# NVIDIA-Merlin/distributed-embeddings

Measured on NVIDIA H100. Metric: DLRM global samples/sec (device-timed, max over ranks), higher is better.
Workload: dtype bf16

## Files before the change

distributed_embeddings_b200/models/dlrm_fast.py:

```python
from __future__ import annotations

import os
from typing import Optional

import torch
from torch import nn

from ..ops import _native
from ..parallel.comm import CommContext
from ..parallel.fused import FusedEngine
from ..utils import nvtx
from ..utils.lr_schedule import LearningRateScheduler
from ..utils.metrics import BinnedAUC, auc_from_histogram
from .dense_optimizer import FlatDenseOptimizer, dense_optimizer_config
from .dlrm import DLRM


def _pad8(n: int) -> int:
  return (n + 7) // 8 * 8


class _Layer:

  def __init__(self, lin: nn.Linear, relu: bool):
    self.lin = lin
    self.relu = relu
    self.out_f, self.in_f = lin.weight.shape
    self.in_pad = _pad8(self.in_f)
    self.w_off = self.b_off = 0
    self.w_numel = self.out_f * self.in_pad
    self.b_numel = _pad8(self.out_f)


class DLRMTrainStep:

  def __init__(self, model: DLRM, lr: float = 24.0, embedding_optimizer: str = "sgd",
               scheduler: Optional[LearningRateScheduler] = None, use_cuda_graph: bool = True,
               embedding_optimizer_kwargs: Optional[dict] = None, overlap: bool = True,
               gemm: str = "cublas", eval_thresholds: int = 8000, dense_optimizer: str = "sgd",
               dense_optimizer_kwargs: Optional[dict] = None):
    if gemm not in ("cublas", "fused_dgrad", "tcgen05", "tcgen05_pair"):
      raise ValueError("gemm must be cublas | fused_dgrad | tcgen05 | tcgen05_pair")
    self.gemm = gemm
    self.dense_cfg = dense_optimizer_config(dense_optimizer, dense_optimizer_kwargs)
    self.model = model
    self.emb = model.embedding
    if self.emb.backend != "fused":
      raise ValueError("DLRMTrainStep needs the fused embedding back end")
    self.dev = self.emb.device
    self.ops = _native.require()
    self.world = self.emb.world_size
    self.ctx = CommContext.for_group(self.emb.group, self.dev)
    self.scheduler = scheduler
    self.use_cuda_graph = use_cuda_graph
    self.overlap = overlap
    self.emb.set_optimizer(embedding_optimizer, lr=lr, **(embedding_optimizer_kwargs or {}))
    if self.emb._engine is None:
      self.emb._engine = FusedEngine(self.emb)
    self.engine: FusedEngine = self.emb._engine
    self.n_emb = len(model.table_sizes)
    self.dim = model.embedding_dim
    sp_env = os.environ.get("DE_B200_STREAM_PUSH", "auto")
    self._stream_push = self.world > 1 and (sp_env == "1" or (sp_env == "auto" and self.world >= 4))
    self._push_stream = torch.cuda.Stream(device=self.dev) if self._stream_push else None
    self._push_ready = torch.cuda.Event() if self._stream_push else None

# ... 178 lines not shown
    H = self.head
    ops.head_loss(last.y, H.w16.view(-1), H.b16, self.lab_in, 1.0 / b, last.dy,
                  H.gw.view(-1), H.gb, last.gb, self.loss, None)
    for i in range(len(self.top) - 1, -1, -1):
      L = self.top[i]
      x = self.top[i - 1].y if i > 0 else self.z
      dx = self.top[i - 1].dy if i > 0 else self.dz
      self._wgrad(L, x)
      if i > 0:
        self._dgrad_relu(L, x, dx, self.top[i - 1].gb)
      else:
        torch.mm(L.dy, L.w16, out=dx)
    if self._ar_stream is not None:
      ar = self._ar_stream
      ar.wait_stream(torch.cuda.current_stream())
      if getattr(self, "_w_used", False):
        ar.wait_stream(self._wstream)
      off = self.top[0].w_off
      with torch.cuda.stream(ar):
        self.ctx.allreduce_(self.gsym, self.n_flat - off, torch.float32, scale=1.0 / self.world,
                            byte_offset=off * 4, max_blocks=32)
    hb = self.bottom[-1]
    pushed = eng.streamed_push
    if pushed:
      eng.push_counters.zero_()
      self._push_ready.record(torch.cuda.current_stream())
      ops.interact_bwd(hb.y, eng.out, self.n_emb, self.dz, hb.dy, 0, 0, 1.0, eng.routes_stage,
                       len(eng.routes_stage_np), [], eng.push_counters, eng.push_chunk_rows)
      self._push_stream.wait_event(self._push_ready)
      with torch.cuda.stream(self._push_stream):
        eng.launch_streamed_push()
    else:
      ops.interact_bwd(hb.y, eng.out, self.n_emb, self.dz, hb.dy, 0, 0, 1.0, eng.routes_all,
                       len(eng.routes_all_np), eng.sync_grad_signal(), None, 0)
    if self._side is not None:
      self._side.wait_stream(torch.cuda.current_stream())
      if pushed:
        self._side.wait_stream(self._push_stream)
      with torch.cuda.stream(self._side):
        eng.backward_inplace()
    else:
      if pushed:
        torch.cuda.current_stream().wait_stream(self._push_stream)
      eng.backward_inplace()
    ops.relu_bwd_bias(hb.dy, hb.y, hb.gb)
    for i in range(len(self.bottom) - 1, -1, -1):
      L = self.bottom[i]
      x = self.bottom[i - 1].y if i > 0 else self.x0
      self._wgrad(L, x)
      if i > 0:
        self._dgrad_relu(L, x, self.bottom[i - 1].dy, self.bottom[i - 1].gb)
    if self._dp_slots and self._side is not None:
      torch.cuda.current_stream().wait_stream(self._side)
    if getattr(self, "_w_used", False):
      torch.cuda.current_stream().wait_stream(self._wstream)
      self._w_used = False
    if self.world > 1:
      if self._ar_stream is not None:
        ar = self._ar_stream
        ar.wait_stream(torch.cuda.current_stream())
        with torch.cuda.stream(ar):
          self.ctx.allreduce_(self.gsym, self.top[0].w_off, torch.float32, scale=1.0 / self.world)
        torch.cuda.current_stream().wait_stream(ar)
      else:
        self.ctx.allreduce_(self.gsym, self.n_flat, torch.float32, scale=1.0 / self.world)
    self.dense_opt.apply(ops, self.p16, self.g32, self.lr_t)
    self._refresh_transposes()
# ... 181 lines not shown
```

distributed_embeddings_b200/ops/csrc/bindings.cpp:

```cpp
#include <ATen/cuda/CUDAContext.h>
#include <c10/cuda/CUDAGuard.h>
#include <c10/cuda/CUDAStream.h>
#include <cuda_runtime.h>
#include <torch/library.h>
#include <torch/torch.h>

#include <cstdlib>
#include <cstring>
#include <mutex>
#include <string>
#include <unordered_map>
#include <vector>

#include "de_b200.h"

namespace {

using at::Tensor;

#define DE_CUDA_CHECK(expr)                                                              \
  do {                                                                                   \
    cudaError_t _e = (expr);                                                             \
    TORCH_CHECK(_e == cudaSuccess, "CUDA error in " #expr ": ", cudaGetErrorString(_e)); \
  } while (0)
// ... 714 lines not shown
  check_bf16_2d(bottom, "bottom");
  check_bf16_2d(emb, "emb");
  check_bf16_2d(z, "z");
  c10::cuda::CUDAGuard guard(bottom.device());
  const int64_t dim = bottom.size(1);
  TORCH_CHECK(emb.size(1) == n_emb * dim, "emb must be [batch, n_emb * dim]");
  TORCH_CHECK(emb.size(0) >= bottom.size(0) && z.size(0) >= bottom.size(0),
              "emb and z need a row per row of bottom");
  check_row_alignment(bottom, 16, "bottom");
  check_row_alignment(emb, 16, "emb");
  const int64_t need = (n_emb + 1) * n_emb / 2 + dim;
  TORCH_CHECK(z.size(1) >= need, "z is too narrow");
  bool ok = de::launch_interact_fwd(bottom.data_ptr(), bottom.stride(0), emb.data_ptr(),
                                    emb.stride(0), static_cast<int>(n_emb), static_cast<int>(dim),
                                    z.data_ptr(), z.stride(0), static_cast<int>(z.size(1)),
                                    bottom.size(0), sm_count(), cur_stream(), to_sync(sync));
  TORCH_CHECK(ok, "unsupported interaction shape (n_emb <= 31, dim in {16,32,64,128})");
  check_launch();
}

void interact_bwd(const Tensor& bottom, const Tensor& emb, int64_t n_emb, const Tensor& dz,
                  Tensor dbottom, int64_t demb_ptr, int64_t demb_stride, double emb_grad_scale,
                  const c10::optional<Tensor>& routes, int64_t n_routes, at::IntArrayRef sync,
                  const c10::optional<Tensor>& done_counters, int64_t chunk_rows) {
  check_bf16_2d(bottom, "bottom");
  check_bf16_2d(emb, "emb");
  check_bf16_2d(dz, "dz");
  check_bf16_2d(dbottom, "dbottom");
  if (routes.has_value()) {
    TORCH_CHECK(routes->is_cuda() && routes->scalar_type() == at::kByte &&
                routes->numel() >= n_routes * static_cast<int64_t>(sizeof(de::GradRoute)));
  } else {
    TORCH_CHECK(demb_ptr != 0, "interact_bwd needs an embedding-gradient buffer or routes");
  }
  const int64_t dim = bottom.size(1);
  const int64_t batch = bottom.size(0);
  TORCH_CHECK(emb.size(1) == n_emb * dim, "emb must be [batch, n_emb * dim]");
  TORCH_CHECK((n_emb + 1) * n_emb / 2 + dim <= dz.size(1), "dz is too narrow");
  TORCH_CHECK(dbottom.size(1) == dim, "dbottom must be [batch, dim]");
  TORCH_CHECK(emb.size(0) >= batch && dz.size(0) >= batch && dbottom.size(0) >= batch,
              "emb, dz and dbottom need a row per row of bottom");
  check_row_alignment(bottom, 16, "bottom");
  check_row_alignment(emb, 16, "emb");
  check_row_alignment(dbottom, 4, "dbottom");
  if (!routes.has_value())
    TORCH_CHECK(demb_stride % 2 == 0 && demb_ptr % 4 == 0,
                "embedding-gradient rows must start on 4-byte boundaries");
  if (done_counters.has_value()) {
    TORCH_CHECK(done_counters->is_cuda() && done_counters->scalar_type() == at::kInt &&
                    done_counters->is_contiguous(),
                "done_counters must be a contiguous int32 CUDA tensor");
    TORCH_CHECK(chunk_rows > 0, "chunk_rows must be positive with done_counters");
    TORCH_CHECK(done_counters->numel() >= (batch + chunk_rows - 1) / chunk_rows,
                "done_counters needs one counter per chunk of chunk_rows samples");
  }
  c10::cuda::CUDAGuard guard(bottom.device());
  bool ok = de::launch_interact_bwd(bottom.data_ptr(), bottom.stride(0), emb.data_ptr(),
                                    emb.stride(0), static_cast<int>(n_emb), static_cast<int>(dim),
                                    dz.data_ptr(), dz.stride(0), dbottom.data_ptr(),
                                    dbottom.stride(0), reinterpret_cast<void*>(demb_ptr),
                                    demb_stride, static_cast<float>(emb_grad_scale),
                                    bottom.size(0), sm_count(), cur_stream(),
                                    routes.has_value()
                                        ? reinterpret_cast<const de::GradRoute*>(routes->data_ptr())
                                        : nullptr,
                                    static_cast<int>(n_routes), to_sync(sync),
                                    done_counters.has_value()
                                        ? reinterpret_cast<uint32_t*>(done_counters->data_ptr<int>())
                                        : nullptr,
                                    static_cast<int>(chunk_rows));
  TORCH_CHECK(ok, "unsupported interaction shape (n_emb <= 31, dim in {32,64,128}; routed / "
                  "signalling launches need dim in {64,128} and 16-byte aligned rows)");
  check_launch();
}

void avgpool_fwd(const Tensor& x, int64_t n, Tensor out, int64_t stride) {
  check_bf16_2d(x, "x");
  check_bf16_2d(out, "out");
  const int64_t out_len = (n + stride - 1) / stride;
  TORCH_CHECK(x.size(1) >= n && out.size(1) >= out_len && out.size(0) == x.size(0));
  const int64_t pad = std::max<int64_t>(0, (out_len - 1) * stride + stride - n);
  c10::cuda::CUDAGuard guard(x.device());
  de::launch_avgpool_fwd(x.data_ptr(), x.stride(0), static_cast<int>(n), out.data_ptr(),
                         out.stride(0), static_cast<int>(out_len), static_cast<int>(stride),
                         static_cast<int>(pad / 2), x.size(0), cur_stream());
  check_launch();
}

void avgpool_bwd(const Tensor& dout, Tensor dx, int64_t n, int64_t stride) {
  check_bf16_2d(dout, "dout");
  check_bf16_2d(dx, "dx");
  const int64_t out_len = (n + stride - 1) / stride;
  TORCH_CHECK(dx.size(1) >= n && dout.size(1) >= out_len && dout.size(0) == dx.size(0));
// ... 327 lines not shown
      "-> ()",
      &push_grad);
  m.def(
      "stream_push(int[] src_ptrs, int[] dst_ptrs, int[] row_bytes, Tensor counters, "
      "int chunk_rows, int rows, int blocks, int[] sync) -> ()",
      &stream_push);
  m.def(
      "rowslice_reduce(Tensor partial, int out_ptr, int out_stride, int out_dtype, Tensor cols) "
      "-> ()",
      &rowslice_reduce);
  m.def(
      "gather_ragged(Tensor segs, int[] val_ptrs, int[] split_ptrs, Tensor(a!) dst_vals, "
      "Tensor(b!) goff, int b, int max_cap) -> ()",
      &gather_ragged);
  m.def("select_copy(Tensor[] src0, Tensor[] src1, Tensor(a!)[] dst, Tensor slot_flag) -> ()",
        &select_copy);
  m.def("copy_cast_2d(Tensor src, int dst_ptr, int dst_stride, int dst_dtype, float scale) -> ()",
        &copy_cast_2d);
  m.def("interact_fwd(Tensor bottom, Tensor emb, int n_emb, Tensor(a!) z, int[] sync) -> ()",
        &interact_fwd);
  m.def(
      "interact_bwd(Tensor bottom, Tensor emb, int n_emb, Tensor dz, Tensor(a!) dbottom, "
      "int demb_ptr, int demb_stride, float emb_grad_scale, Tensor? routes, int n_routes, "
      "int[] sync, Tensor? done_counters, int chunk_rows) -> ()",
      &interact_bwd);
  m.def("avgpool_fwd(Tensor x, int n, Tensor(a!) out, int stride) -> ()", &avgpool_fwd);
  m.def("avgpool_bwd(Tensor dout, Tensor(a!) dx, int n, int stride) -> ()", &avgpool_bwd);
  m.def("relu_bwd_bias(Tensor(a!) dy, Tensor y, Tensor(b!) db) -> ()", &relu_bwd_bias);
  m.def(
      "head_loss(Tensor x, Tensor w, Tensor bias, Tensor labels, float inv_batch, Tensor(a!) dx, "
      "Tensor(b!) dw, Tensor(c!) db, Tensor(d!) dbias_prev, Tensor(e!) loss_sum, Tensor? logits) "
      "-> ()",
      &head_loss);
  m.def(
      "head_eval(Tensor x, Tensor w, Tensor bias, Tensor labels, Tensor n_valid, Tensor(a!) probs, "
      "Tensor(b!) hist, Tensor(c!) loss_sum, Tensor(d!) count) -> ()",
      &head_eval);
  m.def(
      "dense_sgd(Tensor(a!) p32, Tensor(b!) p16, Tensor(c!) g32, Tensor lr, float grad_scale) "
      "-> ()",
      &dense_sgd);
  m.def(
      "dense_adagrad(Tensor(a!) p32, Tensor(b!) p16, Tensor(c!) g32, Tensor(d!) acc, Tensor lr, "
      "float eps) -> ()",
      &dense_adagrad);
  m.def(
      "dense_adam(Tensor(a!) p32, Tensor(b!) p16, Tensor(c!) g32, Tensor(d!) m, Tensor(e!) v, "
// ... 18 lines not shown
```

distributed_embeddings_b200/ops/csrc/de_b200.h:

```cpp
#pragma once
#include <cuda_runtime.h>
#include <stdint.h>

namespace de {

constexpr int kMaxPeers = 16;
constexpr int kGridCapSms = 132;

struct alignas(16) InputDesc {
  const void* table;
  const void* ids;
  const int64_t* offsets;
  int64_t ids_off;
  int64_t id_shift;
  int64_t sub_rows;
  int64_t row_base;
  int32_t width;
  int32_t hotness;
  int32_t dst_col;
  int32_t combiner;
  int32_t local_table;
  int32_t flags;
  int64_t item_off;
};
// ... 139 lines not shown
};
void launch_stream_push(const PushPlan& plan, const uint32_t* counters, int chunk_rows,
                        int64_t rows, unsigned long long timeout, int* error_flag, int blocks,
                        cudaStream_t stream, const SyncArgs& sync);
void launch_rowslice_reduce(const float* partial, int world, int64_t rows, int64_t part_stride,
                            void* out, int64_t out_stride, int out_dtype, const int32_t* cols,
                            int n_cols, cudaStream_t stream);
void launch_gather_segments(const int64_t* segs, int n_seg, const PeerPtrs& src, void* dst,
                            int elem_bytes, int64_t max_seg_elems, cudaStream_t stream);
void launch_gather_ragged(const int64_t* segs, int n_seg, const PeerPtrs& src_vals,
                          const PeerPtrs& src_splits, void* dst_vals, int64_t* goff, int64_t b,
                          int world, int elem_bytes, int64_t max_cap, cudaStream_t stream);
void launch_select_copy(const void* const* src0, const void* const* src1, void* const* dst,
                        const int64_t* nbytes, int count, const int* slot_flag, int sm_count,
                        cudaStream_t stream);
void launch_copy_cast_2d(const void* src, int64_t src_stride, void* dst, int64_t dst_stride,
                         int64_t rows, int64_t cols, int src_dtype, int dst_dtype, float scale,
                         cudaStream_t stream);

bool launch_interact_fwd(const void* bottom, int64_t bottom_stride, const void* emb,
                         int64_t emb_stride, int n_emb, int dim, void* z, int64_t z_stride,
                         int z_width, int64_t batch, int sm_count, cudaStream_t stream,
                         const SyncArgs& sync);
bool launch_interact_bwd(const void* bottom, int64_t bottom_stride, const void* emb,
                         int64_t emb_stride, int n_emb, int dim, const void* dz,
                         int64_t dz_stride, void* dbottom, int64_t dbottom_stride, void* demb,
                         int64_t demb_stride, float emb_grad_scale, int64_t batch, int sm_count,
                         cudaStream_t stream, const GradRoute* routes, int n_routes,
                         const SyncArgs& sync, uint32_t* done_counters = nullptr,
                         int chunk_rows = 0);
void launch_avgpool_fwd(const void* x, int64_t x_stride, int n, void* out, int64_t out_stride,
                        int out_len, int stride, int left, int64_t rows, cudaStream_t stream);
void launch_avgpool_bwd(const void* dout, int64_t dout_stride, int out_len, void* dx,
                        int64_t dx_stride, int n, int stride, int left, int64_t rows,
                        cudaStream_t stream);
void launch_relu_bwd_bias(void* dy, const void* y, float* db, int64_t rows, int cols,
                          cudaStream_t stream);
bool launch_head_loss(const void* x, int K, const void* w, const void* bias, const float* labels,
                      int64_t batch, float inv_batch, void* dx, float* dw, float* db,
                      float* dbias_prev, float* loss_sum, float* logits_out, int sm_count,
                      cudaStream_t stream);
bool launch_head_eval(const void* x, int K, const void* w, const void* bias, const float* labels,
                      int64_t batch, const int64_t* n_valid, float* probs, int64_t* hist, int nb,
                      double* loss_sum, int64_t* count, int sm_count, cudaStream_t stream);
void launch_sgd_update(float* p32, void* p16, float* g32, const float* lr_ptr, float grad_scale,
                       int64_t n, int sm_count, cudaStream_t stream);
bool launch_dense_opt(int kind, float* p32, void* p16, float* g32, float* s0, float* s1,
                      const float* lr_ptr, const float* step_ptr, float beta1, float beta2,
                      float eps, int64_t n, int sm_count, cudaStream_t stream);
void launch_cast_pad(const float* src, int src_cols, void* dst, int dst_cols, int64_t rows,
                     cudaStream_t stream);

bool launch_gemm_tn_fused(const void* A, int64_t lda, const void* B, int64_t ldb, const void* bias,
// ... 9 lines not shown
```

distributed_embeddings_b200/ops/csrc/dense_kernels.cu:

```cuda
#include <cuda_bf16.h>
#include <cuda_runtime.h>
#include <stdint.h>

#include <cstdlib>

#include "common.cuh"
#include "de_b200.h"

namespace de {

namespace {

using bf16 = __nv_bfloat16;

__device__ __forceinline__ uint32_t smem_u32(const void* p) {
  return static_cast<uint32_t>(__cvta_generic_to_shared(p));
}

__device__ __forceinline__ void ldmatrix_x4(uint32_t (&r)[4], uint32_t addr) {
  asm volatile("ldmatrix.sync.aligned.m8n8.x4.shared.b16 {%0,%1,%2,%3}, [%4];"
               : "=r"(r[0]), "=r"(r[1]), "=r"(r[2]), "=r"(r[3])
               : "r"(addr));
}
__device__ __forceinline__ void ldmatrix_x4_trans(uint32_t (&r)[4], uint32_t addr) {
// ... 217 lines not shown

constexpr int kDzMax = 512;

template <int D>
__device__ __forceinline__ void issue_sample(bf16* sF, int LD, bf16* sDz, const bf16* bottom,
                                             const bf16* emb, const bf16* dz, int n_emb,
                                             int dz_chunks, int lane) {
  constexpr int kChunks = D / 8;
  const int total = (n_emb + 1) * kChunks;
#pragma unroll 4
  for (int c = lane; c < total; c += 32) {
    const int row = c / kChunks, ch = c - row * kChunks;
    const bf16* src = row == 0 ? bottom + ch * 8 : emb + (row - 1) * D + ch * 8;
    cp_async16(sF + row * LD + ch * 8, src);
  }
  for (int c = lane; c < dz_chunks; c += 32) cp_async16(sDz + c * 8, dz + c * 8);
}

struct ChunkDst {
  unsigned long long base;
  long long stride;
};

template <int D>
__global__ void __launch_bounds__(kWarps * 32)
interact_bwd_v2_kernel(const bf16* __restrict__ bottom, int64_t bottom_stride,
                       const bf16* __restrict__ emb, int64_t emb_stride, int n_emb,
                       const bf16* __restrict__ dz, int64_t dz_stride, bf16* __restrict__ dbottom,
                       int64_t dbottom_stride, bf16* __restrict__ demb, int64_t demb_stride,
                       float emb_grad_scale, int64_t batch,
                       const GradRoute* __restrict__ routes, int n_routes,
                       const __grid_constant__ SyncArgs sync, uint32_t* __restrict__ done_counters,
                       int chunk_rows) {
  constexpr int LD = D + 8;
  constexpr int LDG = 40;
  constexpr int kWarpElems = 2 * kMaxFeat * LD + 2 * kDzMax + kMaxFeat * LDG;
  constexpr int kRowChunks = D / 8;
  extern __shared__ __align__(16) unsigned char smem_raw[];
  const int warp = threadIdx.x >> 5, lane = threadIdx.x & 31;
  bf16* base = reinterpret_cast<bf16*>(smem_raw) + warp * kWarpElems;
  bf16* sDz0 = base + 2 * kMaxFeat * LD;
  bf16* sG = sDz0 + 2 * kDzMax;
  ChunkDst* sDst = reinterpret_cast<ChunkDst*>(reinterpret_cast<bf16*>(smem_raw) +
                                               kWarps * kWarpElems);
  const int nf = n_emb + 1;
  const int n_inter = nf * (nf - 1) / 2;
  const int dz_chunks = (n_inter + D + 7) >> 3;
  const int n_chunks = n_emb * kRowChunks;
  if (routes == nullptr) {
    for (int c = threadIdx.x; c < n_chunks; c += blockDim.x) {
      sDst[c].base = reinterpret_cast<unsigned long long>(demb + c * 8);
      sDst[c].stride = demb_stride * 2;
    }
  } else {
    for (int r = 0; r < n_routes; ++r) {
      const GradRoute R = routes[r];
      const int c0 = R.src_col >> 3, nc = R.width >> 3;
      for (int c = threadIdx.x; c < nc; c += blockDim.x) {
        sDst[c0 + c].base =
            reinterpret_cast<unsigned long long>(reinterpret_cast<bf16*>(R.dst) + R.dst_col + c * 8);
        sDst[c0 + c].stride = R.dst_stride * 2;
      }
    }
  }
  zero_pad_rows<D>(base, LD, n_emb, lane);
  zero_pad_rows<D>(base + kMaxFeat * LD, LD, n_emb, lane);
  __syncthreads();

  const int64_t stride = static_cast<int64_t>(gridDim.x) * kWarps;
  int64_t s = static_cast<int64_t>(blockIdx.x) * kWarps + warp;
  int cur = 0;
  if (s < batch)
    issue_sample<D>(base, LD, sDz0, bottom + s * bottom_stride, emb + s * emb_stride,
                    dz + s * dz_stride, n_emb, dz_chunks, lane);
  cp_async_commit();
  for (; s < batch; s += stride, cur ^= 1) {
    const int64_t nxt = s + stride;
    if (nxt < batch)
      issue_sample<D>(base + (cur ^ 1) * (kMaxFeat * LD), LD, sDz0 + (cur ^ 1) * kDzMax,
                      bottom + nxt * bottom_stride, emb + nxt * emb_stride, dz + nxt * dz_stride,
                      n_emb, dz_chunks, lane);
    cp_async_commit();
    cp_async_wait_group<1>();
    __syncwarp();
    bf16* sF = base + cur * (kMaxFeat * LD);
    const bf16* sDz = sDz0 + cur * kDzMax;
    for (int c = lane; c < kMaxFeat * LDG / 8; c += 32)
      reinterpret_cast<uint4*>(sG)[c] = make_uint4(0, 0, 0, 0);
    __syncwarp();
    for (int idx = lane; idx < n_inter; idx += 32) {
      int i = static_cast<int>((1.0f + sqrtf(1.0f + 8.0f * idx)) * 0.5f);
      while (i * (i - 1) / 2 > idx) --i;
      while ((i + 1) * i / 2 <= idx) ++i;
      const int j = idx - i * (i - 1) / 2;
      const bf16 v = sDz[idx];
      sG[i * LDG + j] = v;
      sG[j * LDG + i] = v;
    }
    __syncwarp();
    uint32_t ga[2][2][4];
#pragma unroll
    for (int mt = 0; mt < 2; ++mt)
#pragma unroll
      for (int ks = 0; ks < 2; ++ks)
// ... 22 lines not shown
      for (int mt = 0; mt < 2; ++mt) {
#pragma unroll
        for (int nt = 0; nt < 4; ++nt) {
#pragma unroll
          for (int half = 0; half < 2; ++half) {
            const int row = mt * 16 + cr + half * 8;
            const int col = n0 + nt * 8 + cc;
            float v0 = acc[mt][nt][half * 2], v1 = acc[mt][nt][half * 2 + 1];
            if (row == 0) {
              v0 += __bfloat162float(sDz[n_inter + col]);
              v1 += __bfloat162float(sDz[n_inter + col + 1]);
            } else {
              v0 *= emb_grad_scale;
              v1 *= emb_grad_scale;
            }
            if (row <= n_emb)
              *reinterpret_cast<__nv_bfloat162*>(sF + row * LD + col) =
                  __floats2bfloat162_rn(v0, v1);
          }
        }
      }
    }
    __syncwarp();
    if (lane < kRowChunks)
      *reinterpret_cast<uint4*>(dbottom + s * dbottom_stride + lane * 8) =
          *reinterpret_cast<const uint4*>(sF + lane * 8);
    for (int c = lane; c < n_chunks; c += 32) {
      const int row = 1 + c / kRowChunks, ch = c - (row - 1) * kRowChunks;
      const ChunkDst d = sDst[c];
      *reinterpret_cast<uint4*>(d.base + static_cast<unsigned long long>(s * d.stride)) =
          *reinterpret_cast<const uint4*>(sF + row * LD + ch * 8);
    }
    __syncwarp();
    if (done_counters != nullptr && lane == 0) {
      __threadfence();
      atomicAdd(done_counters + s / chunk_rows, 1u);
    }
  }
  cp_async_wait_group<0>();
  sync_tail(sync);
}

constexpr int kRbUnroll = 4;
__global__ void __launch_bounds__(256)
relu_bwd_bias_kernel(bf16* __restrict__ dy, const bf16* __restrict__ y, float* __restrict__ db,
                     int64_t rows, int cols, int rows_per_block) {
  extern __shared__ float s_part[];
  const int tpr = cols >> 3;
  const int rows_par = blockDim.x / tpr;
  const int tr = threadIdx.x / tpr, tc = threadIdx.x - tr * tpr;
  const int64_t r0 = static_cast<int64_t>(blockIdx.x) * rows_per_block;
  const int64_t r1 = min(rows, r0 + rows_per_block);
  float acc[8] = {0, 0, 0, 0, 0, 0, 0, 0};
  if (tr < rows_par) {
    for (int64_t r = r0 + tr; r < r1; r += static_cast<int64_t>(rows_par) * kRbUnroll) {
      uint4 g[kRbUnroll], a[kRbUnroll];
#pragma unroll
      for (int u = 0; u < kRbUnroll; ++u) {
        const int64_t rr = r + static_cast<int64_t>(u) * rows_par;
        if (rr < r1) {
          g[u] = *reinterpret_cast<const uint4*>(dy + rr * cols + tc * 8);
          a[u] = *reinterpret_cast<const uint4*>(y + rr * cols + tc * 8);
        }
// ... 328 lines not shown
#define DE_IFWD(DD)                                                                              \
  {                                                                                              \
    const size_t smem = kWarps * fwd_warp_bytes(DD);                                             \
    cudaFuncSetAttribute(interact_fwd_kernel<DD>, cudaFuncAttributeMaxDynamicSharedMemorySize,   \
                         static_cast<int>(smem));                                                \
    interact_fwd_kernel<DD><<<static_cast<unsigned>(blocks), kWarps * 32, smem, stream>>>(       \
        reinterpret_cast<const bf16*>(bottom), bottom_stride, reinterpret_cast<const bf16*>(emb), \
        emb_stride, n_emb, reinterpret_cast<bf16*>(z), z_stride, z_width, batch, sync);          \
    return true;                                                                                 \
  }
  if (dim == 128) DE_IFWD(128)
  if (dim == 64) DE_IFWD(64)
  if (dim == 32) DE_IFWD(32)
  if (dim == 16) DE_IFWD(16)
#undef DE_IFWD
  return false;
}

bool launch_interact_bwd(const void* bottom, int64_t bottom_stride, const void* emb,
                         int64_t emb_stride, int n_emb, int dim, const void* dz,
                         int64_t dz_stride, void* dbottom, int64_t dbottom_stride, void* demb,
                         int64_t demb_stride, float emb_grad_scale, int64_t batch, int sm_count,
                         cudaStream_t stream, const GradRoute* routes, int n_routes,
                         const SyncArgs& sync, uint32_t* done_counters, int chunk_rows) {
  if (n_emb + 1 > kMaxFeat || batch <= 0 || dim % 32 != 0) return false;
  int64_t blocks = (batch + kWarps - 1) / kWarps;
  const int64_t cap = static_cast<int64_t>(sm_count) * 8;
  if (blocks > cap) blocks = cap;
  static const bool force_v1 = [] {
    const char* v = std::getenv("DE_B200_INTERACT_V1");
    return v != nullptr && v[0] == '1';
  }();
  const int nf = n_emb + 1;
  const int dz_elems = (nf * (nf - 1) / 2 + dim + 7) / 8 * 8;
  const bool v2_ok =
      dz_elems <= kDzMax && dz_elems <= dz_stride && dz_stride % 8 == 0 &&
      bottom_stride % 8 == 0 && emb_stride % 8 == 0 && dbottom_stride % 8 == 0 &&
      ((reinterpret_cast<uintptr_t>(dz) | reinterpret_cast<uintptr_t>(bottom) |
        reinterpret_cast<uintptr_t>(emb) | reinterpret_cast<uintptr_t>(dbottom)) & 15) == 0 &&
      (dim == 128 || dim == 64) &&
      (routes != nullptr || (demb_stride % 8 == 0 && (reinterpret_cast<uintptr_t>(demb) & 15) == 0));
  if ((routes != nullptr || done_counters != nullptr) && !v2_ok) return false;
  const bool has_sync = sync.state != nullptr && (sync.wait_ch >= 0 || sync.signal_ch >= 0);
  if (v2_ok && (!force_v1 || routes != nullptr || has_sync || done_counters != nullptr)) {
    int64_t blocks2 = (batch + kWarps - 1) / kWarps;
    if (blocks2 > static_cast<int64_t>(sm_count) * 2) blocks2 = static_cast<int64_t>(sm_count) * 2;
#define DE_IBWD2(DD)                                                                             \
  {                                                                                              \
    const size_t smem =                                                                          \
        kWarps * (2 * kMaxFeat * (DD + 8) + 2 * kDzMax + kMaxFeat * 40) * sizeof(bf16) +         \
        static_cast<size_t>(n_emb) * (DD / 8) * sizeof(ChunkDst);                                \
    cudaFuncSetAttribute(interact_bwd_v2_kernel<DD>,                                             \
                         cudaFuncAttributeMaxDynamicSharedMemorySize, static_cast<int>(smem));   \
    interact_bwd_v2_kernel<DD><<<static_cast<unsigned>(blocks2), kWarps * 32, smem, stream>>>(   \
        reinterpret_cast<const bf16*>(bottom), bottom_stride, reinterpret_cast<const bf16*>(emb), \
        emb_stride, n_emb, reinterpret_cast<const bf16*>(dz), dz_stride,                         \
        reinterpret_cast<bf16*>(dbottom), dbottom_stride, reinterpret_cast<bf16*>(demb),         \
        demb_stride, emb_grad_scale, batch, routes, n_routes, sync, done_counters, chunk_rows);  \
    return true;                                                                                 \
  }
    if (dim == 128) DE_IBWD2(128)
    if (dim == 64) DE_IBWD2(64)
#undef DE_IBWD2
  }
  if (has_sync) return false;
#define DE_IBWD(DD)                                                                              \
  {                                                                                              \
    const size_t smem = kWarps * (kMaxFeat * (DD + 8) + kMaxFeat * 40) * sizeof(bf16);           \
    cudaFuncSetAttribute(interact_bwd_kernel<DD>, cudaFuncAttributeMaxDynamicSharedMemorySize,   \
                         static_cast<int>(smem));                                                \
    interact_bwd_kernel<DD><<<static_cast<unsigned>(blocks), kWarps * 32, smem, stream>>>(       \
        reinterpret_cast<const bf16*>(bottom), bottom_stride, reinterpret_cast<const bf16*>(emb), \
        emb_stride, n_emb, reinterpret_cast<const bf16*>(dz), dz_stride,                         \
        reinterpret_cast<bf16*>(dbottom), dbottom_stride, reinterpret_cast<bf16*>(demb),         \
        demb_stride, emb_grad_scale, batch);                                                     \
    return true;                                                                                 \
  }
  if (dim == 128) DE_IBWD(128)
  if (dim == 64) DE_IBWD(64)
  if (dim == 32) DE_IBWD(32)
#undef DE_IBWD
  return false;
}

void launch_relu_bwd_bias(void* dy, const void* y, float* db, int64_t rows, int cols,
// ... 104 lines not shown
```

distributed_embeddings_b200/parallel/dry_run.py:

```python
from __future__ import annotations

import bisect
import ctypes
import threading
from typing import Dict, List, Optional, Sequence, Tuple

import numpy as np
import torch

from ..ops._native import GRAD_ROUTE, INPUT_DESC, MAX_PEERS, TABLE_DESC
from ..ops.stochastic_rounding import stochastic_round
from . import fused as _fused


class DryWorld:

  def __init__(self, world_size: int):
    self.world_size = int(world_size)
    self.lock = threading.Lock()
    self._barrier = threading.Barrier(self.world_size)
    self._bufs: Dict[Tuple[int, int], torch.Tensor] = {}
    self._ranges: Dict[int, int] = {}
    self._starts: List[int] = []
    self._keep: List[torch.Tensor] = []
# ... 336 lines not shown
    self._count("scatter_add_bwd")
    self._wait(sync)
    if staged:
      esz = 4 if int(act_dtype) == 0 else 2
      assert (grad_stride * esz) % 16 == 0 and all(int(p) % 16 == 0 for p in grad_ptrs)
      for d in self._descs(descs, n_inputs):
        rb = int(d["width"]) * esz
        assert rb % 16 == 0 and rb <= 256 and (int(d["dst_col"]) * esz) % 16 == 0
    if scale_ptr:
      scale = scale * float(self.world.tensor(int(scale_ptr), torch.float32, 1, "lr")[0])
    for d in self._descs(descs, n_inputs):
      table = self._table(d)
      for dd in range(-(-batch // grad_batch)):
        g0, g1 = dd * grad_batch, min(batch, (dd + 1) * grad_batch)
        vals, lens = self._ids_of(d, g0, g1, ids64, src_ptrs, src_batch)
        ids = vals + int(d["id_shift"])
        ok = (ids >= 0) & (ids < int(d["sub_rows"]))
        g = self._grad_rows(d, dd, g1 - g0, grad_ptrs, grad_stride, act_dtype)
        w = torch.full((g1 - g0,), float(scale))
        if int(d["combiner"]) == 1:
          w = w / lens.clamp(min=1).to(w.dtype)
        per_id = (g * w.unsqueeze(1))[self._pool_index(lens)]
        table.index_add_(0, int(d["row_base"]) + ids[ok], per_id[ok])

  def sort_items(self, descs, tables, n_tables, n_inputs, batch, src_batch, src_ptrs, ids64,
                 n_items, total_rows, prefill_sentinel):
    self._count("sort_items")
    D = self._descs(descs, n_inputs)
    T = self._descs(tables, n_tables, TABLE_DESC)
    keys = torch.full((n_items,), int(total_rows), dtype=torch.int64)
    items = torch.zeros(n_items, dtype=torch.int64)
    covered = torch.zeros(n_items, dtype=torch.bool)
    for f, d in enumerate(D):
      vals, lens = self._ids_of(d, 0, batch, ids64, src_ptrs, src_batch)
      ids = vals + int(d["id_shift"])
      ok = (ids >= 0) & (ids < int(d["sub_rows"]))
      key = int(T[int(d["local_table"])]["key_base"]) + int(d["row_base"]) + ids
      key = torch.where(ok, key, torch.full_like(key, int(total_rows)))
      first = int(d["item_off"])
      if int(d["offsets"]):
        offs = self.world.tensor(int(d["offsets"]), torch.int64, batch + 1, "csr offsets")
        first += int(offs[0])
      n = key.numel()
      assert first + n <= n_items, "item range outside the sort buffers"
      assert not bool(covered[first:first + n].any()), "item ranges of two inputs overlap"
      covered[first:first + n] = True
# ... 152 lines not shown
```

distributed_embeddings_b200/parallel/fused.py:

```python
from __future__ import annotations

import os
import weakref
from typing import Any, Dict, List, Optional, Sequence, Tuple

import numpy as np
import torch

from ..ops import _native
from ..ops._native import DTYPE_CODE, GRAD_ROUTE, INPUT_DESC, TABLE_DESC
from ..ops.ragged import RaggedIds
from ..utils import nvtx
from .comm import CH_BARRIER0, CH_CONSUMED, CH_GRAD, CH_IDS, CH_OUT, CommContext

_OPT_KIND = {"sgd": _native.OPT_SGD, "adagrad": _native.OPT_ADAGRAD,
             "rowwise_adagrad": _native.OPT_ROWWISE_ADAGRAD, "adam": _native.OPT_ADAM}
_COMB = {None: 0, "sum": 0, "mean": 1}

FLAG_SKIP_EMPTY = 1
FLAG_CATCH_LOW = 2
FLAG_CATCH_HIGH = 4


def _weight(layer):
  return layer.embeddings


def _dev_ptr(t: torch.Tensor) -> int:
  if t.is_cuda:
    return t.data_ptr()
  if not t.is_pinned():
    raise RuntimeError("host-resident tables must live in pinned memory for the fused back end")
  return int(_native.require().host_device_pointer(t))


class _FusedFn(torch.autograd.Function):

  @staticmethod
  def forward(ctx, engine, token, *weights):
    ctx.engine = engine
    ctx.n_weights = len(weights)
    ctx.done = False
    engine._gen += 1
    ctx.gen = engine._gen
    out = engine._run_forward()
    engine._pending = weakref.ref(ctx)
    if not getattr(engine.de, "zero_copy_output", False):
      out = out.clone()
    return out

  @staticmethod
  def backward(ctx, grad_out):
    engine = ctx.engine
    if ctx.gen != engine._gen:
      raise RuntimeError(
          "DistributedEmbedding (fused back end): another forward ran on this layer before the "
# ... 758 lines not shown
    key = (self._key, tuple(t.data_ptr() for t in self._dp_targets))
    if self._dp_target_desc is None or self._dp_target_desc[0] != key:
      d = self.ddesc_np.copy()
      for j in range(len(d)):
        d[j]["table"] = self._dp_targets[int(d[j]["local_table"])].data_ptr()
      self._dp_target_desc = (key, _native.upload_struct_array(d, self.device), len(d))
    _, dd, n = self._dp_target_desc
    self.ops.scatter_add_bwd(dd, n, self.lb, self.lb, self.lb, self.total_width, [],
                             [self.grad.data_ptr()], 0, 1.0, 0, self.ids64, self.act, self.vec4,
                             False, [], self.staged_dp)

  @property
  def streamed_push(self) -> bool:
    return self.gstage is not None

  def launch_streamed_push(self, blocks: int = 32):
    src, dst, row_bytes = self.push_plan
    self.ops.stream_push(src, dst, row_bytes, self.push_counters, self.push_chunk_rows, self.lb,
                         blocks, self._sync(signal=CH_GRAD))

  def sync_grad_signal(self):
    return self._sync(signal=CH_GRAD) if (self.W > 1 and self.mpdesc is not None) else []

  def backward_inplace(self):
    if len(self.de.dp_layers):
      if getattr(self, "_dp_targets", None) is None:
        raise RuntimeError("backward_inplace needs set_dp_grad_targets() for replicated tables")
      self._scatter_dp_grads()
    self._backward_mp()

  def _backward_mp(self) -> List[Optional[torch.Tensor]]:
    with nvtx.range("emb_backward_update"):
      return self._backward_mp_impl()

  def _backward_mp_impl(self) -> List[Optional[torch.Tensor]]:
    ops, de = self.ops, self.de
    n_mp = len(self.mp_layers)
    if self.mpdesc is None:
      return [None] * n_mp
    multi = self.W > 1
    if not any(_weight(l).requires_grad for l in self.mp_layers):
      if multi:
        ops.sync_only(self._sync(wait=CH_GRAD, signal=CH_CONSUMED))
      return [None] * n_mp
    opt = de._fused_optimizer
    if opt is not None and opt["kind"] != "sgd" and not self.opt_state:
      self.reset_optimizer_state()
    if self._tables_dirty:
      self._refresh_tables()
    B = self.B
    gscale = 0.0 if self._dry_updates else de.mp_grad_scale
    if opt is not None and opt["kind"] == "sgd" and not opt.get("deterministic", False) and \
        not self.has_offload and self.tab == 0:
      ops.scatter_add_bwd(self.mpdesc, self.n_mp_inputs, B, B, B, self.recv_width, [],
                          self.recv_ptr, 0, -gscale, self.lr_t.data_ptr(), self.ids64,
                          self.act, self.vec4, self.vec8,
                          self._sync(wait=CH_GRAD, signal=CH_CONSUMED), self.staged_update)
      return [None] * n_mp
    if multi:
      ops.sync_only(self._sync(wait=CH_GRAD))
    keys, items, seg, n_unique = ops.sort_items(self.mpdesc, self.tdesc, n_mp, self.n_mp_inputs,
                                                B, B, [], self.ids64, self.n_items,
                                                self.total_rows, self.any_ragged)
    if opt is not None:
      if not self._dry_updates:
        self.step_t.add_(1.0)
      kind = _OPT_KIND[opt["kind"]]
      if self._dry_updates and opt["kind"] == "adam":
        kind = _OPT_KIND["sgd"]
      ops.segment_update(self.mpdesc, self.tdesc, n_mp, B, B, self.recv_width, self.recv_ptr,
                         keys, items, seg, n_unique, kind, opt["lr"],
                         opt["eps"], opt["beta1"], opt["beta2"], 1.0, 1.0, gscale,
                         opt["weight_decay"], self.lr_t.data_ptr(), None, None, self.max_width,
                         self.act, self.vec4, self._balanced_scratch(), self.step_t.data_ptr(),
                         self.tab)
      if multi:
        ops.sync_only(self._sync(signal=CH_CONSUMED))
# ... 35 lines not shown
```

Measured before the change: 17.04 million.

## Apply large-table SGD updates directly inside interaction backward kernel

For single-GPU atomic-SGD runs with 128-wide one-hot tables of at least a minimum row count, the interaction backward kernel now adds the scaled embedding gradient straight into the fp32 table rows with red.add atomics. It also prefetches the next sample's table rows into L2. The point is to skip writing bf16 gradients to the receive buffer and reading them back in the separate scatter_add update pass. Only the remaining tables go through scatter_add. The kernel does more atomic traffic on the critical path and adds a specialised kernel variant.

```diff
diff --git a/distributed_embeddings_b200/models/dlrm_fast.py b/distributed_embeddings_b200/models/dlrm_fast.py
--- a/distributed_embeddings_b200/models/dlrm_fast.py
+++ b/distributed_embeddings_b200/models/dlrm_fast.py
@@ -15,6 +15,8 @@
 from .dense_optimizer import FlatDenseOptimizer, dense_optimizer_config
 from .dlrm import DLRM
 
+FUSED_UPDATE_MIN_ROWS = 20000
+
 
 def _pad8(n: int) -> int:
   return (n + 7) // 8 * 8
@@ -38,10 +40,13 @@
                scheduler: Optional[LearningRateScheduler] = None, use_cuda_graph: bool = True,
                embedding_optimizer_kwargs: Optional[dict] = None, overlap: bool = True,
                gemm: str = "cublas", eval_thresholds: int = 8000, dense_optimizer: str = "sgd",
-               dense_optimizer_kwargs: Optional[dict] = None):
+               dense_optimizer_kwargs: Optional[dict] = None, fused_table_update: bool = True,
+               fused_update_min_rows: int = FUSED_UPDATE_MIN_ROWS):
     if gemm not in ("cublas", "fused_dgrad", "tcgen05", "tcgen05_pair"):
       raise ValueError("gemm must be cublas | fused_dgrad | tcgen05 | tcgen05_pair")
     self.gemm = gemm
+    self.fused_table_update = bool(fused_table_update)
+    self.fused_update_min_rows = int(fused_update_min_rows)
     self.dense_cfg = dense_optimizer_config(dense_optimizer, dense_optimizer_kwargs)
     self.model = model
     self.emb = model.embedding
@@ -266,6 +271,7 @@
                             byte_offset=off * 4, max_blocks=32)
     hb = self.bottom[-1]
     pushed = eng.streamed_push
+    applied = None
     if pushed:
       eng.push_counters.zero_()
       self._push_ready.record(torch.cuda.current_stream())
@@ -275,18 +281,21 @@
       with torch.cuda.stream(self._push_stream):
         eng.launch_streamed_push()
     else:
+      applied = eng.producer_update(self.dim, self.fused_update_min_rows) \
+          if self.fused_table_update else None
       ops.interact_bwd(hb.y, eng.out, self.n_emb, self.dz, hb.dy, 0, 0, 1.0, eng.routes_all,
-                       len(eng.routes_all_np), eng.sync_grad_signal(), None, 0)
+                       len(eng.routes_all_np), eng.sync_grad_signal(), None, 0,
+                       *(applied.interact_args() if applied else ()))
     if self._side is not None:
       self._side.wait_stream(torch.cuda.current_stream())
       if pushed:
         self._side.wait_stream(self._push_stream)
       with torch.cuda.stream(self._side):
-        eng.backward_inplace()
+        eng.backward_inplace(applied)
     else:
       if pushed:
         torch.cuda.current_stream().wait_stream(self._push_stream)
-      eng.backward_inplace()
+      eng.backward_inplace(applied)
     ops.relu_bwd_bias(hb.dy, hb.y, hb.gb)
     for i in range(len(self.bottom) - 1, -1, -1):
       L = self.bottom[i]
diff --git a/distributed_embeddings_b200/ops/csrc/bindings.cpp b/distributed_embeddings_b200/ops/csrc/bindings.cpp
--- a/distributed_embeddings_b200/ops/csrc/bindings.cpp
+++ b/distributed_embeddings_b200/ops/csrc/bindings.cpp
@@ -760,7 +760,43 @@
 void interact_bwd(const Tensor& bottom, const Tensor& emb, int64_t n_emb, const Tensor& dz,
                   Tensor dbottom, int64_t demb_ptr, int64_t demb_stride, double emb_grad_scale,
                   const c10::optional<Tensor>& routes, int64_t n_routes, at::IntArrayRef sync,
-                  const c10::optional<Tensor>& done_counters, int64_t chunk_rows) {
+                  const c10::optional<Tensor>& done_counters, int64_t chunk_rows,
+                  const c10::optional<Tensor>& apply_descs, double apply_scale,
+                  int64_t apply_scale_ptr, bool apply_ids64) {
+  de::InteractApply apply{};
+  if (apply_descs.has_value()) {
+    const Tensor& a = *apply_descs;
+    TORCH_CHECK(!a.is_cuda() && a.scalar_type() == at::kByte && a.is_contiguous(),
+                "apply_descs must be a contiguous uint8 CPU tensor of InputDesc records");
+    TORCH_CHECK(a.numel() == n_emb * static_cast<int64_t>(sizeof(de::InputDesc)),
+                "apply_descs needs one InputDesc per embedding row");
+    TORCH_CHECK(n_emb <= de::kMaxInteractApply, "apply_descs: at most 31 embedding rows");
+    TORCH_CHECK(apply_scale_ptr % 4 == 0, "apply_scale_ptr must be 4-byte aligned");
+    TORCH_CHECK(!done_counters.has_value(), "apply_descs cannot be combined with done_counters");
+    const auto* d = reinterpret_cast<const de::InputDesc*>(a.data_ptr());
+    for (int64_t f = 0; f < n_emb; ++f) {
+      if (d[f].table == nullptr) continue;
+      TORCH_CHECK(d[f].width == 128 && bottom.size(1) == 128,
+                  "apply_descs: applied tables must be 128 wide, like the interaction");
+      TORCH_CHECK(d[f].hotness == 1 && d[f].offsets == nullptr && d[f].ids != nullptr,
+                  "apply_descs: applied inputs must be one-hot with direct ids");
+      TORCH_CHECK(reinterpret_cast<uintptr_t>(d[f].table) % 16 == 0,
+                  "apply_descs: tables must be 16-byte aligned");
+      TORCH_CHECK(reinterpret_cast<uintptr_t>(d[f].ids) % (apply_ids64 ? 8 : 4) == 0,
+                  "apply_descs: ids must be aligned to their element size");
+      TORCH_CHECK(d[f].row_base >= 0 && d[f].sub_rows >= 0,
+                  "apply_descs: row_base and sub_rows must not be negative");
+      apply.table[f] = static_cast<float*>(const_cast<void*>(d[f].table));
+      apply.ids[f] = d[f].ids;
+      apply.row_base[f] = d[f].row_base;
+      apply.sub_rows[f] = d[f].sub_rows;
+      apply.id_shift[f] = d[f].id_shift;
+      apply.mask |= 1u << f;
+    }
+    apply.scale = static_cast<float>(apply_scale);
+    apply.scale_ptr = reinterpret_cast<const float*>(apply_scale_ptr);
+    apply.ids64 = apply_ids64 ? 1 : 0;
+  }
   check_bf16_2d(bottom, "bottom");
   check_bf16_2d(emb, "emb");
   check_bf16_2d(dz, "dz");
@@ -806,7 +842,8 @@
                                     done_counters.has_value()
                                         ? reinterpret_cast<uint32_t*>(done_counters->data_ptr<int>())
                                         : nullptr,
-                                    static_cast<int>(chunk_rows));
+                                    static_cast<int>(chunk_rows),
+                                    apply.mask != 0 ? &apply : nullptr);
   TORCH_CHECK(ok, "unsupported interaction shape (n_emb <= 31, dim in {32,64,128}; routed / "
                   "signalling launches need dim in {64,128} and 16-byte aligned rows)");
   check_launch();
@@ -1180,7 +1217,8 @@
   m.def(
       "interact_bwd(Tensor bottom, Tensor emb, int n_emb, Tensor dz, Tensor(a!) dbottom, "
       "int demb_ptr, int demb_stride, float emb_grad_scale, Tensor? routes, int n_routes, "
-      "int[] sync, Tensor? done_counters, int chunk_rows) -> ()",
+      "int[] sync, Tensor? done_counters, int chunk_rows, Tensor? apply_descs=None, "
+      "float apply_scale=0.0, int apply_scale_ptr=0, bool apply_ids64=False) -> ()",
       &interact_bwd);
   m.def("avgpool_fwd(Tensor x, int n, Tensor(a!) out, int stride) -> ()", &avgpool_fwd);
   m.def("avgpool_bwd(Tensor dout, Tensor(a!) dx, int n, int stride) -> ()", &avgpool_bwd);
diff --git a/distributed_embeddings_b200/ops/csrc/de_b200.h b/distributed_embeddings_b200/ops/csrc/de_b200.h
--- a/distributed_embeddings_b200/ops/csrc/de_b200.h
+++ b/distributed_embeddings_b200/ops/csrc/de_b200.h
@@ -185,13 +185,26 @@
                          int64_t emb_stride, int n_emb, int dim, void* z, int64_t z_stride,
                          int z_width, int64_t batch, int sm_count, cudaStream_t stream,
                          const SyncArgs& sync);
+constexpr int kMaxInteractApply = 31;
+struct InteractApply {
+  float* table[kMaxInteractApply];
+  const void* ids[kMaxInteractApply];
+  int64_t row_base[kMaxInteractApply];
+  int64_t sub_rows[kMaxInteractApply];
+  int64_t id_shift[kMaxInteractApply];
+  const float* scale_ptr;
+  float scale;
+  uint32_t mask;
+  int32_t ids64;
+};
+
 bool launch_interact_bwd(const void* bottom, int64_t bottom_stride, const void* emb,
                          int64_t emb_stride, int n_emb, int dim, const void* dz,
                          int64_t dz_stride, void* dbottom, int64_t dbottom_stride, void* demb,
                          int64_t demb_stride, float emb_grad_scale, int64_t batch, int sm_count,
                          cudaStream_t stream, const GradRoute* routes, int n_routes,
                          const SyncArgs& sync, uint32_t* done_counters = nullptr,
-                         int chunk_rows = 0);
+                         int chunk_rows = 0, const InteractApply* apply = nullptr);
 void launch_avgpool_fwd(const void* x, int64_t x_stride, int n, void* out, int64_t out_stride,
                         int out_len, int stride, int left, int64_t rows, cudaStream_t stream);
 void launch_avgpool_bwd(const void* dout, int64_t dout_stride, int out_len, void* dx,
diff --git a/distributed_embeddings_b200/ops/csrc/dense_kernels.cu b/distributed_embeddings_b200/ops/csrc/dense_kernels.cu
--- a/distributed_embeddings_b200/ops/csrc/dense_kernels.cu
+++ b/distributed_embeddings_b200/ops/csrc/dense_kernels.cu
@@ -263,16 +263,19 @@
   long long stride;
 };
 
-template <int D>
-__global__ void __launch_bounds__(kWarps * 32)
-interact_bwd_v2_kernel(const bf16* __restrict__ bottom, int64_t bottom_stride,
-                       const bf16* __restrict__ emb, int64_t emb_stride, int n_emb,
-                       const bf16* __restrict__ dz, int64_t dz_stride, bf16* __restrict__ dbottom,
-                       int64_t dbottom_stride, bf16* __restrict__ demb, int64_t demb_stride,
-                       float emb_grad_scale, int64_t batch,
-                       const GradRoute* __restrict__ routes, int n_routes,
-                       const __grid_constant__ SyncArgs sync, uint32_t* __restrict__ done_counters,
-                       int chunk_rows) {
+__device__ __forceinline__ void prefetch_l2(const void* p) {
+  asm volatile("prefetch.global.L2 [%0];" ::"l"(p));
+}
+
+template <int D, bool APPLY>
+__device__ __forceinline__ void
+interact_bwd_v2_body(const bf16* __restrict__ bottom, int64_t bottom_stride,
+                     const bf16* __restrict__ emb, int64_t emb_stride, int n_emb,
+                     const bf16* __restrict__ dz, int64_t dz_stride, bf16* __restrict__ dbottom,
+                     int64_t dbottom_stride, bf16* __restrict__ demb, int64_t demb_stride,
+                     float emb_grad_scale, int64_t batch, const GradRoute* __restrict__ routes,
+                     int n_routes, const SyncArgs& sync, uint32_t* __restrict__ done_counters,
+                     int chunk_rows, const InteractApply& apply) {
   constexpr int LD = D + 8;
   constexpr int LDG = 40;
   constexpr int kWarpElems = 2 * kMaxFeat * LD + 2 * kDzMax + kMaxFeat * LDG;
@@ -308,19 +311,53 @@
   zero_pad_rows<D>(base + kMaxFeat * LD, LD, n_emb, lane);
   __syncthreads();
 
+  float apply_scale = 0.f;
+  long long id_cur = -1, id_next = -1;
+  if constexpr (APPLY) {
+    apply_scale = apply.scale;
+    if (apply.scale_ptr != nullptr) apply_scale *= *apply.scale_ptr;
+  }
+  auto load_id = [&](int64_t smp) -> long long {
+    if (lane < n_emb && ((apply.mask >> lane) & 1u)) {
+      const long long raw = apply.ids64 ? static_cast<const int64_t*>(apply.ids[lane])[smp]
+                                        : static_cast<const int32_t*>(apply.ids[lane])[smp];
+      const long long id = raw + apply.id_shift[lane];
+      if (static_cast<unsigned long long>(id) < static_cast<unsigned long long>(apply.sub_rows[lane]))
+        return id;
+    }
+    return -1;
+  };
+  auto prefetch_row = [&](long long id) {
+    if (id >= 0) {
+      const char* row = reinterpret_cast<const char*>(apply.table[lane] +
+                                                      (apply.row_base[lane] + id) * D);
+#pragma unroll
+      for (int l = 0; l < D * 4 / 128; ++l) prefetch_l2(row + (l << 7));
+    }
+  };
+
   const int64_t stride = static_cast<int64_t>(gridDim.x) * kWarps;
   int64_t s = static_cast<int64_t>(blockIdx.x) * kWarps + warp;
   int cur = 0;
-  if (s < batch)
+  if (s < batch) {
     issue_sample<D>(base, LD, sDz0, bottom + s * bottom_stride, emb + s * emb_stride,
                     dz + s * dz_stride, n_emb, dz_chunks, lane);
+    if constexpr (APPLY) {
+      id_cur = load_id(s);
+      prefetch_row(id_cur);
+    }
+  }
   cp_async_commit();
   for (; s < batch; s += stride, cur ^= 1) {
     const int64_t nxt = s + stride;
-    if (nxt < batch)
+    if (nxt < batch) {
       issue_sample<D>(base + (cur ^ 1) * (kMaxFeat * LD), LD, sDz0 + (cur ^ 1) * kDzMax,
                       bottom + nxt * bottom_stride, emb + nxt * emb_stride, dz + nxt * dz_stride,
                       n_emb, dz_chunks, lane);
+      if constexpr (APPLY) id_next = load_id(nxt);
+    } else if constexpr (APPLY) {
+      id_next = -1;
+    }
     cp_async_commit();
     cp_async_wait_group<1>();
     __syncwarp();
@@ -389,14 +426,46 @@
       }
     }
     __syncwarp();
+    if constexpr (APPLY) prefetch_row(id_next);
     if (lane < kRowChunks)
       *reinterpret_cast<uint4*>(dbottom + s * dbottom_stride + lane * 8) =
           *reinterpret_cast<const uint4*>(sF + lane * 8);
-    for (int c = lane; c < n_chunks; c += 32) {
-      const int row = 1 + c / kRowChunks, ch = c - (row - 1) * kRowChunks;
-      const ChunkDst d = sDst[c];
-      *reinterpret_cast<uint4*>(d.base + static_cast<unsigned long long>(s * d.stride)) =
-          *reinterpret_cast<const uint4*>(sF + row * LD + ch * 8);
+    if constexpr (APPLY) {
+      for (int c0 = 0; c0 < n_chunks; c0 += 32) {
+        const int c = c0 + lane;
+        const int f = c / kRowChunks, ch = c - f * kRowChunks;
+        const long long id = __shfl_sync(0xffffffffu, id_cur, f & 31);
+        if (c >= n_chunks) continue;
+        const uint4 v = *reinterpret_cast<const uint4*>(sF + (f + 1) * LD + ch * 8);
+        if ((apply.mask >> f) & 1u) {
+          if (id >= 0) {
+            const __nv_bfloat162* h = reinterpret_cast<const __nv_bfloat162*>(&v);
+            FVec<4> lo, hi;
+#pragma unroll
+            for (int k = 0; k < 2; ++k) {
+              const float2 a = __bfloat1622float2(h[k]), b = __bfloat1622float2(h[k + 2]);
+              lo.v[2 * k] = a.x * apply_scale;
+              lo.v[2 * k + 1] = a.y * apply_scale;
+              hi.v[2 * k] = b.x * apply_scale;
+              hi.v[2 * k + 1] = b.y * apply_scale;
+            }
+            float* dst = apply.table[f] + (apply.row_base[f] + id) * D + ch * 8;
+            red_add_f32<4>(dst, lo);
+            red_add_f32<4>(dst + 4, hi);
+          }
+        } else {
+          const ChunkDst d = sDst[c];
+          *reinterpret_cast<uint4*>(d.base + static_cast<unsigned long long>(s * d.stride)) = v;
+        }
+      }
+      id_cur = id_next;
+    } else {
+      for (int c = lane; c < n_chunks; c += 32) {
+        const int row = 1 + c / kRowChunks, ch = c - (row - 1) * kRowChunks;
+        const ChunkDst d = sDst[c];
+        *reinterpret_cast<uint4*>(d.base + static_cast<unsigned long long>(s * d.stride)) =
+            *reinterpret_cast<const uint4*>(sF + row * LD + ch * 8);
+      }
     }
     __syncwarp();
     if (done_counters != nullptr && lane == 0) {
@@ -406,6 +475,37 @@
   }
   cp_async_wait_group<0>();
   sync_tail(sync);
+}
+
+template <int D>
+__global__ void __launch_bounds__(kWarps * 32)
+interact_bwd_v2_kernel(const bf16* __restrict__ bottom, int64_t bottom_stride,
+                       const bf16* __restrict__ emb, int64_t emb_stride, int n_emb,
+                       const bf16* __restrict__ dz, int64_t dz_stride, bf16* __restrict__ dbottom,
+                       int64_t dbottom_stride, bf16* __restrict__ demb, int64_t demb_stride,
+                       float emb_grad_scale, int64_t batch,
+                       const GradRoute* __restrict__ routes, int n_routes,
+                       const __grid_constant__ SyncArgs sync, uint32_t* __restrict__ done_counters,
+                       int chunk_rows) {
+  interact_bwd_v2_body<D, false>(bottom, bottom_stride, emb, emb_stride, n_emb, dz, dz_stride,
+                                 dbottom, dbottom_stride, demb, demb_stride, emb_grad_scale, batch,
+                                 routes, n_routes, sync, done_counters, chunk_rows,
+                                 InteractApply{});
+}
+
+template <int D>
+__global__ void __launch_bounds__(kWarps * 32)
+interact_bwd_apply_kernel(const bf16* __restrict__ bottom, int64_t bottom_stride,
+                          const bf16* __restrict__ emb, int64_t emb_stride, int n_emb,
+                          const bf16* __restrict__ dz, int64_t dz_stride,
+                          bf16* __restrict__ dbottom, int64_t dbottom_stride,
+                          bf16* __restrict__ demb, int64_t demb_stride, float emb_grad_scale,
+                          int64_t batch, const GradRoute* __restrict__ routes, int n_routes,
+                          const __grid_constant__ SyncArgs sync,
+                          const __grid_constant__ InteractApply apply) {
+  interact_bwd_v2_body<D, true>(bottom, bottom_stride, emb, emb_stride, n_emb, dz, dz_stride,
+                                dbottom, dbottom_stride, demb, demb_stride, emb_grad_scale, batch,
+                                routes, n_routes, sync, nullptr, 0, apply);
 }
 
 constexpr int kRbUnroll = 4;
@@ -780,8 +880,11 @@
                          int64_t dz_stride, void* dbottom, int64_t dbottom_stride, void* demb,
                          int64_t demb_stride, float emb_grad_scale, int64_t batch, int sm_count,
                          cudaStream_t stream, const GradRoute* routes, int n_routes,
-                         const SyncArgs& sync, uint32_t* done_counters, int chunk_rows) {
+                         const SyncArgs& sync, uint32_t* done_counters, int chunk_rows,
+                         const InteractApply* apply) {
   if (n_emb + 1 > kMaxFeat || batch <= 0 || dim % 32 != 0) return false;
+  const bool applied = apply != nullptr && apply->mask != 0;
+  if (applied && (dim != 128 || done_counters != nullptr)) return false;
   int64_t blocks = (batch + kWarps - 1) / kWarps;
   const int64_t cap = static_cast<int64_t>(sm_count) * 8;
   if (blocks > cap) blocks = cap;
@@ -798,27 +901,29 @@
         reinterpret_cast<uintptr_t>(emb) | reinterpret_cast<uintptr_t>(dbottom)) & 15) == 0 &&
       (dim == 128 || dim == 64) &&
       (routes != nullptr || (demb_stride % 8 == 0 && (reinterpret_cast<uintptr_t>(demb) & 15) == 0));
-  if ((routes != nullptr || done_counters != nullptr) && !v2_ok) return false;
+  if ((routes != nullptr || done_counters != nullptr || applied) && !v2_ok) return false;
   const bool has_sync = sync.state != nullptr && (sync.wait_ch >= 0 || sync.signal_ch >= 0);
-  if (v2_ok && (!force_v1 || routes != nullptr || has_sync || done_counters != nullptr)) {
+  if (v2_ok &&
+      (!force_v1 || routes != nullptr || has_sync || done_counters != nullptr || applied)) {
     int64_t blocks2 = (batch + kWarps - 1) / kWarps;
     if (blocks2 > static_cast<int64_t>(sm_count) * 2) blocks2 = static_cast<int64_t>(sm_count) * 2;
-#define DE_IBWD2(DD)                                                                             \
+#define DE_IBWD2(KERNEL, DD, ...)                                                                \
   {                                                                                              \
     const size_t smem =                                                                          \
         kWarps * (2 * kMaxFeat * (DD + 8) + 2 * kDzMax + kMaxFeat * 40) * sizeof(bf16) +         \
         static_cast<size_t>(n_emb) * (DD / 8) * sizeof(ChunkDst);                                \
-    cudaFuncSetAttribute(interact_bwd_v2_kernel<DD>,                                             \
-                         cudaFuncAttributeMaxDynamicSharedMemorySize, static_cast<int>(smem));   \
-    interact_bwd_v2_kernel<DD><<<static_cast<unsigned>(blocks2), kWarps * 32, smem, stream>>>(   \
+    cudaFuncSetAttribute(KERNEL<DD>, cudaFuncAttributeMaxDynamicSharedMemorySize,                \
+                         static_cast<int>(smem));                                                \
+    KERNEL<DD><<<static_cast<unsigned>(blocks2), kWarps * 32, smem, stream>>>(                   \
         reinterpret_cast<const bf16*>(bottom), bottom_stride, reinterpret_cast<const bf16*>(emb), \
         emb_stride, n_emb, reinterpret_cast<const bf16*>(dz), dz_stride,                         \
         reinterpret_cast<bf16*>(dbottom), dbottom_stride, reinterpret_cast<bf16*>(demb),         \
-        demb_stride, emb_grad_scale, batch, routes, n_routes, sync, done_counters, chunk_rows);  \
+        demb_stride, emb_grad_scale, batch, routes, n_routes, sync, __VA_ARGS__);                \
     return true;                                                                                 \
   }
-    if (dim == 128) DE_IBWD2(128)
-    if (dim == 64) DE_IBWD2(64)
+    if (applied) DE_IBWD2(interact_bwd_apply_kernel, 128, *apply)
+    if (dim == 128) DE_IBWD2(interact_bwd_v2_kernel, 128, done_counters, chunk_rows)
+    if (dim == 64) DE_IBWD2(interact_bwd_v2_kernel, 64, done_counters, chunk_rows)
 #undef DE_IBWD2
   }
   if (has_sync) return false;
diff --git a/distributed_embeddings_b200/parallel/dry_run.py b/distributed_embeddings_b200/parallel/dry_run.py
--- a/distributed_embeddings_b200/parallel/dry_run.py
+++ b/distributed_embeddings_b200/parallel/dry_run.py
@@ -382,6 +382,23 @@
           w = w / lens.clamp(min=1).to(w.dtype)
         per_id = (g * w.unsqueeze(1))[self._pool_index(lens)]
         table.index_add_(0, int(d["row_base"]) + ids[ok], per_id[ok])
+
+  def interact_bwd_apply(self, demb, apply_descs, scale, scale_ptr, ids64):
+    self._count("interact_bwd_apply")
+    if scale_ptr:
+      scale = scale * float(self.world.tensor(int(scale_ptr), torch.float32, 1, "lr")[0])
+    batch = demb.shape[0]
+    for f, d in enumerate(self._descs(apply_descs, apply_descs.numel() // INPUT_DESC.itemsize)):
+      if not int(d["table"]):
+        continue
+      assert int(d["width"]) == 128 and int(d["hotness"]) == 1 and not int(d["offsets"]) and \
+          int(d["ids"]), "applied inputs are one-hot, direct ids, 128 wide"
+      table = self._table(d)
+      vals, _ = self._ids_of(d, 0, batch, ids64, [], batch)
+      ids = vals + int(d["id_shift"])
+      ok = (ids >= 0) & (ids < int(d["sub_rows"]))
+      g = demb[:, f * 128:(f + 1) * 128].float() * float(scale)
+      table.index_add_(0, int(d["row_base"]) + ids[ok], g[ok])
 
   def sort_items(self, descs, tables, n_tables, n_inputs, batch, src_batch, src_ptrs, ids64,
                  n_items, total_rows, prefill_sentinel):
diff --git a/distributed_embeddings_b200/parallel/fused.py b/distributed_embeddings_b200/parallel/fused.py
--- a/distributed_embeddings_b200/parallel/fused.py
+++ b/distributed_embeddings_b200/parallel/fused.py
@@ -2,7 +2,7 @@
 
 import os
 import weakref
-from typing import Any, Dict, List, Optional, Sequence, Tuple
+from typing import Any, Dict, List, NamedTuple, Optional, Sequence, Tuple
 
 import numpy as np
 import torch
@@ -32,6 +32,19 @@
   if not t.is_pinned():
     raise RuntimeError("host-resident tables must live in pinned memory for the fused back end")
   return int(_native.require().host_device_pointer(t))
+
+
+class ProducerUpdate(NamedTuple):
+  mpdesc: torch.Tensor
+  apply_descs: torch.Tensor
+  scale: float
+  scale_ptr: int
+  ids64: bool
+  rest_descs: Optional[torch.Tensor]
+  n_rest: int
+
+  def interact_args(self) -> tuple:
+    return self.apply_descs, self.scale, self.scale_ptr, self.ids64
 
 
 class _FusedFn(torch.autograd.Function):
@@ -836,19 +849,57 @@
   def sync_grad_signal(self):
     return self._sync(signal=CH_GRAD) if (self.W > 1 and self.mpdesc is not None) else []
 
-  def backward_inplace(self):
+  def backward_inplace(self, producer: Optional["ProducerUpdate"] = None):
     if len(self.de.dp_layers):
       if getattr(self, "_dp_targets", None) is None:
         raise RuntimeError("backward_inplace needs set_dp_grad_targets() for replicated tables")
       self._scatter_dp_grads()
-    self._backward_mp()
-
-  def _backward_mp(self) -> List[Optional[torch.Tensor]]:
+    self._backward_mp(producer)
+
+  def _atomic_sgd(self) -> bool:
+    opt = self.de._fused_optimizer
+    return opt is not None and opt["kind"] == "sgd" and not opt.get("deterministic", False) and \
+        not self.has_offload and self.tab == 0
+
+  def producer_update(self, dim: int, min_rows: int) -> Optional["ProducerUpdate"]:
+    if self._key is None or self.W != 1 or not self._atomic_sgd() or not self.vec4 or \
+        self.any_ragged or dim != 128 or self.mpdesc is None or \
+        not any(_weight(l).requires_grad for l in self.mp_layers):
+      return None
+    cache = getattr(self, "_producer_split", None)
+    if cache is None or cache[0] != (self._key, dim, min_rows) or cache[1] is not self.mpdesc:
+      n_feat = len(self.out_cols) - 1
+      apply = np.zeros(n_feat, dtype=INPUT_DESC)
+      taken = np.zeros(self.n_mp_inputs, dtype=bool)
+      if self.out_cols == [dim * f for f in range(n_feat + 1)] and n_feat <= 31:
+        for i, d in enumerate(self.cdesc_np):
+          f, off = divmod(int(d["dst_col"]), dim)
+          if off == 0 and int(d["width"]) == dim and int(d["hotness"]) == 1 and \
+              int(d["offsets"]) == 0 and int(d["ids"]) != 0 and int(d["sub_rows"]) >= min_rows:
+            apply[f] = d
+            taken[i] = True
+      rest = self.mpdesc_np[~taken]
+      rest_dev = _native.upload_struct_array(rest, self.device) if len(rest) else None
+      apply_t = torch.from_numpy(apply.view(np.uint8).copy()) if taken.any() else None
+      self._producer_split = ((self._key, dim, min_rows), self.mpdesc, apply_t, rest_dev, len(rest))
+    _, mpdesc, apply_t, rest_dev, n_rest = self._producer_split
+    if apply_t is None:
+      return None
+    gscale = 0.0 if self._dry_updates else self.de.mp_grad_scale
+    return ProducerUpdate(mpdesc, apply_t, -gscale, self.lr_t.data_ptr(), self.ids64, rest_dev,
+                          n_rest)
+
+  def _backward_mp(self, producer: Optional["ProducerUpdate"] = None
+                   ) -> List[Optional[torch.Tensor]]:
     with nvtx.range("emb_backward_update"):
-      return self._backward_mp_impl()
-
-  def _backward_mp_impl(self) -> List[Optional[torch.Tensor]]:
+      return self._backward_mp_impl(producer)
+
+  def _backward_mp_impl(self, producer: Optional["ProducerUpdate"] = None
+                        ) -> List[Optional[torch.Tensor]]:
     ops, de = self.ops, self.de
+    if producer is not None and (producer.mpdesc is not self.mpdesc or not self._atomic_sgd()):
+      raise ValueError("the producer update was built for another plan or optimizer: call "
+                       "producer_update() for the current one")
     n_mp = len(self.mp_layers)
     if self.mpdesc is None:
       return [None] * n_mp
@@ -864,9 +915,13 @@
       self._refresh_tables()
     B = self.B
     gscale = 0.0 if self._dry_updates else de.mp_grad_scale
-    if opt is not None and opt["kind"] == "sgd" and not opt.get("deterministic", False) and \
-        not self.has_offload and self.tab == 0:
-      ops.scatter_add_bwd(self.mpdesc, self.n_mp_inputs, B, B, B, self.recv_width, [],
+    if self._atomic_sgd():
+      descs, n = self.mpdesc, self.n_mp_inputs
+      if producer is not None:
+        descs, n = producer.rest_descs, producer.n_rest
+        if n == 0:
+          return [None] * n_mp
+      ops.scatter_add_bwd(descs, n, B, B, B, self.recv_width, [],
                           self.recv_ptr, 0, -gscale, self.lr_t.data_ptr(), self.ids64,
                           self.act, self.vec4, self.vec8,
                           self._sync(wait=CH_GRAD, signal=CH_CONSUMED), self.staged_update)
```

Result: faster. 17.90 million, median of 6 (+5.0%).
